# alex-ozdemir/collaborative-zksnark

Measured on AMD Instinct MI355X. Metric: collaborative Groth16 proofs/sec (BLS12-377, 2^20 constraints, SPDZ N=2), higher is better.
Workload: dtype u32

## Files before the change

collaborative-zksnark_amd/csrc/core.hip:

```cpp
#include <string.h>
#include "czk_internal.h"

#include <stdlib.h>
#include <unistd.h>

namespace {
struct HwQueueDefault {
    HwQueueDefault() { setenv("GPU_MAX_HW_QUEUES", "8", 0); }
} g_hw_queue_default;
}

namespace czk {

int set_err(czk_ctx* ctx, int code, const std::string& msg) {
    if (ctx) ctx->err = msg;
    return code;
}

int ensure_buf(czk_ctx* ctx, DeviceBuf& b, size_t bytes) {
    if (b.bytes >= bytes) return CZK_OK;
    if (b.p) {
        CZK_HIP(ctx, hipStreamSynchronize(ctx->stream));
        CZK_HIP(ctx, hipFree(b.p));
        b.p = nullptr;
// ... 340 lines not shown
    (void)hipSetDevice(ctx->device);
    (void)hipStreamSynchronize(ctx->stream);
    for (auto& kv : ctx->domains) {
        DomainTables& d = kv.second;
        if (d.tw_fwd) (void)hipFree(d.tw_fwd);
        if (d.tw_inv) (void)hipFree(d.tw_inv);
        if (d.coset_fwd) (void)hipFree(d.coset_fwd);
        if (d.coset_inv) (void)hipFree(d.coset_inv);
        if (d.twu_fwd) (void)hipFree(d.twu_fwd);
        if (d.twu_inv) (void)hipFree(d.twu_inv);
        if (d.cosetu_fwd) (void)hipFree(d.cosetu_fwd);
        if (d.cosetu_inv) (void)hipFree(d.cosetu_inv);
    }
    for (auto& kv : ctx->mixed_domains) {
        MixedDomain& d = kv.second;
        if (d.tw_fwd) (void)hipFree(d.tw_fwd);
        if (d.tw_inv) (void)hipFree(d.tw_inv);
        if (d.coset_fwd) (void)hipFree(d.coset_fwd);
        if (d.coset_inv) (void)hipFree(d.coset_inv);
    }
    if (ctx->mixed_scratch.p) (void)hipFree(ctx->mixed_scratch.p);
    if (ctx->ntt_scratch.p) (void)hipFree(ctx->ntt_scratch.p);
    if (ctx->poly_scratch.p) (void)hipFree(ctx->poly_scratch.p);
    if (ctx->open_bad) (void)hipFree(ctx->open_bad);
    for (auto& b : ctx->stage_pool) (void)hipFree(b.p);
    ctx->stage_pool.clear();
    if (ctx->share_tab.p) (void)hipFree(ctx->share_tab.p);
    msm_pipeline_destroy(ctx);
    xfer_destroy(ctx);
    prof_resolve(ctx);
    for (hipEvent_t e : ctx->event_pool) (void)hipEventDestroy(e);
    if (ctx->prof_base) (void)hipEventDestroy(ctx->prof_base);
    if (ctx->own_stream) (void)hipStreamDestroy(ctx->stream);
    delete ctx;
}

namespace {
struct OptDesc {
    const char* name;
    long lo, hi;
    bool before_pipeline;
    void (*set)(czk_ctx*, long);
};
const OptDesc OPTIONS[] = {
    {"msm_slots", 1, czk_ctx::MSM_SLOTS, true, [](czk_ctx* c, long v) { c->msm_slots_in_use = (int)v; }},
    {"msm_stream_priority", 0, 2, true, [](czk_ctx* c, long v) { c->msm_stream_prio = (int)v; }},
    {"msm_lane_interleave", 0, 64, false, [](czk_ctx* c, long v) { c->msm_lane_interleave = (int)v; }},
    {"msm_sort_reuse", 0, 1, false, [](czk_ctx* c, long v) { c->msm_sort_reuse = v != 0; }},
    {"msm_sort_onepass", 0, 1, false, [](czk_ctx* c, long v) { c->msm_sort_onepass = v != 0; }},
    {"msm_fixed_c", 0, 1, false, [](czk_ctx* c, long v) { c->msm_fixed_c = v != 0; }},
    {"msm_window_g1", 0, 22, false, [](czk_ctx* c, long v) { c->msm_c_g1 = (unsigned)v; }},
    {"msm_window_g2", 0, 22, false, [](czk_ctx* c, long v) { c->msm_c_g2 = (unsigned)v; }},
    {"ntt_gen1", 0, 1, false, [](czk_ctx* c, long v) { c->ntt_gen1 = v != 0; }},
    {"ntt_fuse_pairs", 0, 1, false, [](czk_ctx* c, long v) { c->ntt_fuse_pairs = v != 0; }},
    {"net_create_timeout_ms", 0, 3600000, false, [](czk_ctx* c, long v) { c->net_create_timeout_ms = v; }},
#ifdef CZK_LAB
    {"msm_affine_rounds", 0, 3, false, [](czk_ctx* c, long v) { c->msm_affine_rounds = (unsigned)v; }},
    {"msm_reduce_sat", 0, 1, false, [](czk_ctx* c, long v) { c->msm_reduce_sat = v != 0; }},
    {"msm_reduce_sat_g2", 0, 1, false, [](czk_ctx* c, long v) { c->msm_reduce_sat_g2 = v != 0; }},
    {"msm_g2_mode", 0, 2, false, [](czk_ctx* c, long v) { c->msm_g2_mode = (int)v; }},
    {"msm_sat", 0, 1, false, [](czk_ctx* c, long v) { c->msm_sat = v != 0; }},
    {"msm_sat_g2", 0, 1, false, [](czk_ctx* c, long v) { c->msm_sat_g2 = v != 0; }},
    {"msm_no_te", 0, 1, false, [](czk_ctx* c, long v) { c->msm_no_te = v != 0; }},
    {"chaos", 0, 0x7fffffff, false, [](czk_ctx* c, long v) { c->chaos = v ? ((unsigned long long)v * 0x9E3779B97F4A7C15ull) ^ ((unsigned long long)getpid() << 32) ^ (unsigned long long)(uintptr_t)c : 0; }},
    {"chaos_drop_wait", 0, 1, false, [](czk_ctx* c, long v) { c->chaos_drop_wait = (int)v; }},
    {"ntt_skip_coset_first", 0, 1, false, [](czk_ctx* c, long v) { c->ntt_skip_coset_first = v != 0; }},
    {"msm_sort_reuse_any_inf", 0, 1, false, [](czk_ctx* c, long v) { c->msm_sort_reuse_any_inf = v != 0; }},

#endif
};
}
extern "C" int czk_ctx_set_option(czk_ctx* ctx, const char* name, long value) {
    if (!ctx || !name) return CZK_ERR_ARG;
    for (const OptDesc& o : OPTIONS) {
        if (strcmp(o.name, name) != 0) continue;
        if (value < o.lo || value > o.hi || (!strncmp(name, "msm_window", 10) && value != 0 && value < 8))
            return set_err(ctx, CZK_ERR_ARG, std::string("czk_ctx_set_option: value out of range for ") + name);
        if (o.before_pipeline && ctx->s_sort) return set_err(ctx, CZK_ERR_ARG, std::string("czk_ctx_set_option: ") + name + " must be set before the context's first MSM");
        CZK_HIP(ctx, hipStreamSynchronize(ctx->stream));
        CZK_TRY(msm_pipeline_sync(ctx));
        o.set(ctx, value);
        return CZK_OK;
    }
#ifdef CZK_LAB
    return set_err(ctx, CZK_ERR_ARG, std::string("czk_ctx_set_option: unknown option \"") + name + "\" (lab build)");
#else
    return set_err(ctx, CZK_ERR_ARG, std::string("czk_ctx_set_option: unknown option \"") + name + "\" (product build: the switches of the rejected variants exist in libczk_hip_lab.so only)");
#endif
}
extern "C" int czk_build_is_lab(void) {
#ifdef CZK_LAB
    return 1;
#else
    return 0;
#endif
}

extern "C" int czk_ctx_reserve(czk_ctx* ctx, unsigned ntt_log_d, size_t ntt_lanes, const czk_bases* bases, size_t n_scalars, size_t msm_lanes) {
    if (!ctx) return CZK_ERR_ARG;
    CZK_HIP(ctx, hipSetDevice(ctx->device));
    if (ntt_lanes) CZK_TRY(ntt_reserve(ctx, ntt_log_d, ntt_lanes));
    if (bases && msm_lanes) CZK_TRY(msm_reserve(ctx, bases, n_scalars, msm_lanes));
    return CZK_OK;
}
extern "C" void* czk_ctx_stream(const czk_ctx* ctx) { return ctx ? (void*)ctx->stream : nullptr; }
extern "C" int czk_ctx_sync(czk_ctx* ctx) {
// ... 65 lines not shown
```

collaborative-zksnark_amd/csrc/czk_internal.h:

```cpp
#pragma once
#include <hip/hip_runtime.h>

#include <atomic>
#include <map>
#include <mutex>
#include <string>
#include <vector>

#include "../../include/czk.h"
#include "curve.h"

namespace czk {

struct DomainTables {
    unsigned log_d = 0;
    u64* tw_fwd = nullptr;
    u64* tw_inv = nullptr;
    u64* coset_fwd = nullptr;
    u64* coset_inv = nullptr;
    uint32_t *twu_fwd = nullptr, *twu_inv = nullptr, *cosetu_fwd = nullptr, *cosetu_inv = nullptr;
    Fr size_inv, group_gen, group_gen_inv, generator, generator_inv, vanishing_inv;
};

struct MixedDomain {
// ... 53 lines not shown
    unsigned split_W = 0, c = 0;
    int group = 0;
    size_t lanes = 0;
};
struct CtxMark {
    uint64_t id = 0;
    hipEvent_t ev_stream = nullptr, ev_red = nullptr;
    uint64_t upto = 0;
};
}

#ifndef CZK_ACC_INTERLEAVE_DEFAULT
#define CZK_ACC_INTERLEAVE_DEFAULT 4u
#endif
struct czk_ctx {
    std::vector<czk::DeviceBuf> stage_pool;
    char* xfer_pinned[2] = {nullptr, nullptr};
    hipEvent_t xfer_ev[2] = {nullptr, nullptr};
    bool xfer_busy[2] = {false, false};
    hipStream_t s_sort = nullptr, s_acc = nullptr, s_red = nullptr;
    hipEvent_t ev_in = nullptr;
    static constexpr int MSM_SLOTS = 4;
    czk::MsmSlot msm_slots[MSM_SLOTS];
    int msm_next_slot = 0;
    uint64_t msm_seq = 0, msm_leader_seq = 0;
    int msm_slots_in_use = 4;
    char* msm_pinned = nullptr;
    size_t msm_pinned_bytes = 0, msm_pinned_used = 0;
    std::vector<czk::MsmPending> msm_pending;
    uint64_t msm_delivered = 0;
    std::vector<czk::CtxMark> marks;
    uint64_t next_mark = 1;
    std::vector<hipEvent_t> mark_events;
    bool msm_sort_reuse = false;
    bool msm_sort_reuse_any_inf = false;
    bool msm_sort_onepass = false;
    bool msm_fixed_c = false;
    unsigned msm_c_g1 = 0, msm_c_g2 = 0;
    bool msm_launch_split = false;
    int msm_lane_interleave = 0;
    int msm_stream_prio = 0;
    unsigned msm_affine_rounds = 0;
    bool msm_reduce_sat = false;
    bool msm_reduce_sat_g2 = false;
    int msm_g2_mode = 0;
    bool msm_sat = false, msm_sat_g2 = false;
    bool msm_no_te = false;
    long net_create_timeout_ms = 0;
    unsigned long long* open_bad = nullptr;
    bool ntt_skip_coset_first = false;
    unsigned long long chaos = 0;
    int chaos_drop_wait = 0;
    bool ntt_fuse_pairs = false;
    bool ntt_gen1 = false;
    bool profiling = false;
    std::map<std::string, czk::ProfEntry> prof;
    std::vector<hipEvent_t> event_pool;
    hipEvent_t prof_base = nullptr;
    int device = 0;
    hipStream_t stream = nullptr;
    bool own_stream = false;
    std::string err;
    std::map<unsigned, czk::DomainTables> domains;
    std::map<unsigned, czk::MixedDomain> mixed_domains;
    czk::DeviceBuf mixed_scratch;
    czk::DeviceBuf ntt_scratch;
    czk::DeviceBuf poly_scratch;
    czk::DeviceBuf share_tab;
    int num_cu = 256;
    size_t lds_per_block = 64 * 1024;
};

struct czk_table_set {
    unsigned c = 0, W = 0;
    size_t cover = 0;
    uint64_t* pts = nullptr;
    uint8_t* inf = nullptr;
};

struct czk_bases {
    static constexpr int MAX_EXTRA = 12;
    czk_table_set extra[MAX_EXTRA];
    std::atomic<int> n_extra{0};
    std::atomic<unsigned> nomem_class{0};
    std::mutex build_mu;
    bool per_call_width = true;
    int device = 0;
    int group = 1;
    size_t n = 0;
    unsigned c = 0;
    unsigned W = 0;
    bool unsat = false;
    bool te = false;
    bool check_wanted = false;
    bool checked = false;
    size_t n_bad = 0;
    bool te_wanted = true;
    uint64_t* pts_sw0 = nullptr;
    bool split = false;
    uint64_t* pts = nullptr;
    uint8_t* inf = nullptr;
    static constexpr size_t INF_LIST_MAX = 4096;
    bool inf_listed = false;
    std::vector<uint32_t> inf_idx;
};

// ... 168 lines not shown
```

collaborative-zksnark_amd/csrc/ntt.hip:

```cpp
#include <atomic>
#include <condition_variable>
#include <mutex>
#include <thread>

#include "czk_internal.h"
#include "ntt_pass.h"

namespace czk {

__device__ __forceinline__ Fr lds_get(const uint4* s, unsigned idx) {
    uint4 a = s[2 * idx], b = s[2 * idx + 1];
    Fr r;
    r.l[0] = a.x; r.l[1] = a.y; r.l[2] = a.z; r.l[3] = a.w;
    r.l[4] = b.x; r.l[5] = b.y; r.l[6] = b.z; r.l[7] = b.w;
    return r;
}
__device__ __forceinline__ void lds_put(uint4* s, unsigned idx, const Fr& v) {
    s[2 * idx] = make_uint4(v.l[0], v.l[1], v.l[2], v.l[3]);
    s[2 * idx + 1] = make_uint4(v.l[4], v.l[5], v.l[6], v.l[7]);
}
__device__ __forceinline__ Fr gfr_load(const u64* base, size_t idx) { return fp_load<FrParams>(base + 4 * idx); }
__device__ __forceinline__ void gfr_store(u64* base, size_t idx, const Fr& v) { fp_store<FrParams>(base + 4 * idx, v); }

__device__ __forceinline__ unsigned bitrev(unsigned v, unsigned bits) {
// ... 249 lines not shown
    d.generator_inv = fp_inv(d.generator);
    d.vanishing_inv = fp_inv(fp_sub(fp_pow_u64(d.generator, D), Fr::one()));
    ctx->domains[log_d] = d;
    *out = &ctx->domains[log_d];
    return CZK_OK;
}

constexpr unsigned NTT2_MIN_LOG = 11;

static int ensure_tables(czk_ctx* ctx, DomainTables* d, bool need_coset_fwd, bool need_coset_inv) {
    const unsigned n = d->log_d;
    const size_t D = (size_t)1 << n;
    if ((!d->tw_fwd || !d->tw_inv) && n > 0) {
        StageRoots hr[2];
        for (unsigned s = 0; s < n; s++) {
            Fr wf = d->group_gen, wi = d->group_gen_inv;
            for (unsigned k = 0; k < n - 1 - s; k++) {
                wf = fp_sqr(wf);
                wi = fp_sqr(wi);
            }
            hr[0].w[s] = wf;
            hr[1].w[s] = wi;
        }
        StageRoots* dr = nullptr;
        CZK_HIP(ctx, hipMalloc(&dr, sizeof(hr)));
        CZK_HIP(ctx, hipMemcpyAsync(dr, hr, sizeof(hr), hipMemcpyHostToDevice, ctx->stream));
        if (alloc_table_pair(ctx, &d->tw_fwd, &d->tw_inv, (D - 1 ? D - 1 : 1) * 32) != CZK_OK) {
            (void)hipFree(dr);
            return CZK_ERR_NOMEM;
        }
        size_t chunks = (D - 1 + 63) / 64;
        unsigned blocks = (unsigned)((chunks + 127) / 128);
        hipLaunchKernelGGL(k_twiddle_table, dim3(blocks), dim3(128), 0, ctx->stream, d->tw_fwd, n, dr);
        hipLaunchKernelGGL(k_twiddle_table, dim3(blocks), dim3(128), 0, ctx->stream, d->tw_inv, n, dr + 1);
        hipError_t e = hipGetLastError();
        if (e == hipSuccess) e = hipStreamSynchronize(ctx->stream);
        (void)hipFree(dr);
        if (e != hipSuccess) return drop_table_pair(ctx, &d->tw_fwd, &d->tw_inv, e);
    }
    size_t chunks = (D + 63) / 64;
    unsigned blocks = (unsigned)((chunks + 127) / 128);
    if (need_coset_fwd && !d->coset_fwd) {
        CZK_HIP(ctx, hipMalloc(&d->coset_fwd, D * 32));
        hipLaunchKernelGGL(k_pow_table, dim3(blocks), dim3(128), 0, ctx->stream, d->coset_fwd, D, d->generator, Fr::one());
        CZK_HIP(ctx, hipGetLastError());
    }
    if (need_coset_inv && !d->coset_inv) {
        CZK_HIP(ctx, hipMalloc(&d->coset_inv, D * 32));
        hipLaunchKernelGGL(k_pow_table, dim3(blocks), dim3(128), 0, ctx->stream, d->coset_inv, D, d->generator_inv, d->size_inv);
        CZK_HIP(ctx, hipGetLastError());
    }
    if (n >= NTT2_MIN_LOG) {
        if (!d->twu_fwd || !d->twu_inv) {
            CZK_TRY(alloc_table_pair(ctx, &d->twu_fwd, &d->twu_inv, (D - 1) * 36));
            launch_table_to_u(ctx->stream, d->tw_fwd, D - 1, d->twu_fwd);
            launch_table_to_u(ctx->stream, d->tw_inv, D - 1, d->twu_inv);
            hipError_t e = hipGetLastError();
            if (e != hipSuccess) return drop_table_pair(ctx, &d->twu_fwd, &d->twu_inv, e);
        }
        if (need_coset_fwd && !d->cosetu_fwd) {
            CZK_HIP(ctx, hipMalloc(&d->cosetu_fwd, D * 36));
            launch_table_to_u(ctx->stream, d->coset_fwd, D, d->cosetu_fwd);
            CZK_HIP(ctx, hipGetLastError());
        }
        if (need_coset_inv && !d->cosetu_inv) {
            CZK_HIP(ctx, hipMalloc(&d->cosetu_inv, D * 36));
            launch_table_to_u(ctx->stream, d->coset_inv, D, d->cosetu_inv);
            CZK_HIP(ctx, hipGetLastError());
        }
    }
    return CZK_OK;
}

int ntt_device(czk_ctx* ctx, u64* data, unsigned log_d, size_t lanes, int kind, size_t in_len, const u64* src, size_t src_stride) {
    if (kind < 0 || kind > 3) return set_err(ctx, CZK_ERR_ARG, "bad ntt kind");
    if (!src) {
        src = data;
        src_stride = (size_t)1 << log_d;
    }
    DomainTables* d = nullptr;
    CZK_TRY(get_domain(ctx, log_d, &d));
    const size_t D = (size_t)1 << log_d;
    if (in_len > D) return set_err(ctx, CZK_ERR_SIZE, "coeffs.len() > domain size (radix2/mod.rs:100)");
    if (lanes == 0) return CZK_OK;
    if (log_d > 30) return set_err(ctx, CZK_ERR_SIZE, "domain above 2^30 exceeds this build's table budget");
    const bool inverse = (kind == CZK_IFFT || kind == CZK_COSET_IFFT);
    CZK_TRY(ensure_tables(ctx, d, kind == CZK_COSET_FFT, kind == CZK_COSET_IFFT));

    const unsigned n = log_d;
    unsigned m = n == 0 ? 1 : (n + 6) / 7;
    unsigned groups[8];
    for (unsigned i = 0; i < m; i++) groups[i] = n / m + (i < n % m ? 1 : 0);

    PassArgs a;
    a.tw = inverse ? d->tw_inv : d->tw_fwd;
    a.n = n;
    a.in_len = in_len;
    a.lane_stride = D;
    a.in_lane_stride = src_stride;
    a.postconst = d->size_inv;

    u64* scratch = nullptr;
    if (m > 1) {
        CZK_TRY(ensure_buf(ctx, ctx->ntt_scratch, lanes * D * (n >= NTT2_MIN_LOG ? NTT2_SCRATCH_ELEM_BYTES : 32)));
        scratch = (u64*)ctx->ntt_scratch.p;
    }
    unsigned s_hi_plus1 = n;
    if (n >= NTT2_MIN_LOG && !ctx->ntt_gen1) {
        Pass2Args b;
        b.tw = inverse ? d->twu_inv : d->twu_fwd;
        b.n = n;
        b.in_len = in_len;
        b.lane_stride = D;
        b.in_lane_stride = src_stride;
        b.postconst = host_fr_to_u(d->size_inv);
        for (unsigned p = 0; p < m; p++) {
            const bool first = (p == 0), last = (p == m - 1);
            const unsigned K = groups[p];
            b.s_lo = s_hi_plus1 - K;
// ... 347 lines not shown
```

collaborative-zksnark_amd/csrc/ntt_pass.h:

```cpp
#pragma once
#include "czk_internal.h"
#include "fru.h"

namespace czk {

constexpr int NTT2_SCRATCH_FORMAT = 2;
constexpr bool NTT2_LAZY_SCRATCH = NTT2_SCRATCH_FORMAT == 1;
constexpr bool NTT2_SCRATCH_2R = NTT2_SCRATCH_FORMAT != 0;
constexpr size_t NTT2_SCRATCH_ELEM_BYTES = NTT2_LAZY_SCRATCH ? 36 : 32;

struct Pass2Args {
    const u64* in;
    u64* out;
    const u32* tw;
    const u32* prescale;
    const u32* posttab;
    FrU postconst;
    int post_mode;
    unsigned n;
    unsigned s_lo;
    size_t in_len;
    int first;
    size_t lane_stride;
    size_t in_lane_stride;
};

int launch_ntt2_pass(czk_ctx* ctx, const Pass2Args& a, unsigned K, bool last, size_t lanes);
int launch_ntt2_final_first(czk_ctx* ctx, const Pass2Args& ai, const Pass2Args& af, unsigned C, size_t lanes);
void launch_table_to_u(hipStream_t st, const u64* sat, size_t count, u32* dst);
FrU host_fr_to_u(const Fr& sat);

}
```

collaborative-zksnark_amd/csrc/ntt_pass.hip:

```cpp
#include "ntt_pass.h"

namespace czk {

__device__ __forceinline__ FrU tab_load(const u32* tab, size_t idx) {
    FrU r;
    const u32* p = tab + 9 * idx;
#pragma unroll
    for (int i = 0; i < 9; i++) r.l[i] = p[i];
    return r;
}

template <int K, int U>
__device__ __forceinline__ void bfly(FrU& a, FrU& b, const FrU& w) {
    FrU d = fru_sub<K, U>(a, b);
    a = fru_add(a, b);
    b = fru_mul(d, w);
}

template <int KB>
__device__ __forceinline__ void radix8(FrU* x, const FrU* tw) {
#pragma unroll
    for (int k = 0; k < 4; k++) bfly<KB, 1>(x[k], x[k + 4], tw[k]);
    bfly<2 * KB, 2>(x[0], x[2], tw[4]);
    bfly<2 * KB, 2>(x[1], x[3], tw[5]);
    bfly<2, 1>(x[4], x[6], tw[4]);
    bfly<2, 1>(x[5], x[7], tw[5]);
    x[0] = fru_normalize(x[0]);
    x[1] = fru_normalize(x[1]);
    bfly<4 * KB, 1>(x[0], x[1], tw[6]);
    bfly<2, 1>(x[2], x[3], tw[6]);
    bfly<4, 2>(x[4], x[5], tw[6]);
    bfly<2, 1>(x[6], x[7], tw[6]);
    x[0] = fru_normalize(x[0]);
    x[2] = fru_normalize(x[2]);
    x[4] = fru_normalize(x[4]);
    x[6] = fru_normalize(x[6]);
}
template <int KB>
__device__ __forceinline__ void radix4(FrU* x, const FrU* tw) {
    bfly<KB, 1>(x[0], x[2], tw[0]);
    bfly<KB, 1>(x[1], x[3], tw[1]);
    bfly<2 * KB, 2>(x[0], x[1], tw[2]);
    bfly<2, 1>(x[2], x[3], tw[2]);
    x[0] = fru_normalize(x[0]);
    x[2] = fru_normalize(x[2]);
}

template <int KB>
__device__ __forceinline__ void radix4_last(FrU* x, const FrU& tw1) {
    const FrU d02 = fru_sub<KB, 1>(x[0], x[2]);
    const FrU s02 = fru_add(x[0], x[2]);
    bfly<KB, 1>(x[1], x[3], tw1);
    x[0] = fru_normalize(fru_add(s02, x[1]));
    x[1] = fru_normalize(fru_sub<2 * KB, 2>(s02, x[1]));
    x[2] = fru_normalize(fru_add(d02, x[3]));
    x[3] = fru_normalize(fru_sub<2, 1>(d02, x[3]));
}
template <int KB>
__device__ __forceinline__ void radix8_last(FrU* x, const FrU* tw2, const FrU& tw1) {
    const FrU d04 = fru_sub<KB, 1>(x[0], x[4]);
    x[0] = fru_add(x[0], x[4]);
#pragma unroll
    for (int k = 1; k < 4; k++) bfly<KB, 1>(x[k], x[k + 4], tw2[k]);
    const FrU d = fru_sub<2 * KB, 2>(x[0], x[2]);
    x[0] = fru_add(x[0], x[2]);
    x[2] = d;
    bfly<2 * KB, 2>(x[1], x[3], tw1);
    const FrU e = fru_sub<2, 1>(d04, x[6]);
    x[4] = fru_add(d04, x[6]);
    x[6] = e;
    bfly<2, 1>(x[5], x[7], tw1);
    x[0] = fru_normalize(x[0]);
    x[1] = fru_normalize(x[1]);
    const FrU s01 = fru_add(x[0], x[1]);
    x[1] = fru_normalize(fru_sub<4 * KB, 1>(x[0], x[1]));
    x[0] = fru_normalize(s01);
    const FrU s23 = fru_add(x[2], x[3]);
    x[3] = fru_normalize(fru_sub<2, 1>(x[2], x[3]));
    x[2] = fru_normalize(s23);
    const FrU s45 = fru_add(x[4], x[5]);
    x[5] = fru_normalize(fru_sub<4, 2>(x[4], x[5]));
    x[4] = fru_normalize(s45);
    const FrU s67 = fru_add(x[6], x[7]);
    x[7] = fru_normalize(fru_sub<2, 1>(x[6], x[7]));
    x[6] = fru_normalize(s67);
}

constexpr unsigned NTT2_LOGT = 4, NTT2_T = 16;

template <int NE>
__device__ __forceinline__ FrU lds_get9(const u32* s, unsigned e) {
    FrU r;
#pragma unroll
    for (int i = 0; i < 9; i++) r.l[i] = s[i * NE + e];
    return r;
}
template <int NE>
__device__ __forceinline__ void lds_put9(u32* s, unsigned e, const FrU& v) {
#pragma unroll
    for (int i = 0; i < 9; i++) s[i * NE + e] = v.l[i];
}

template <bool LAZY_IN>
__device__ __forceinline__ FrU load_input(const Pass2Args& a, const u64* in, size_t gi) {
    if constexpr (LAZY_IN && NTT2_LAZY_SCRATCH) return tab_load((const u32*)in, gi);
    if (a.first && gi >= a.in_len) {
        FrU z;
#pragma unroll
        for (int i = 0; i < 9; i++) z.l[i] = 0;
        return z;
    }
    FrU v = fru_unpack(fp_load<FrParams>(in + 4 * gi));
    if (a.prescale) v = fru_mul(v, tab_load(a.prescale, gi));
    return v;
}
__device__ __forceinline__ void store_output(const Pass2Args& a, u64* out, size_t k, const FrU& v, bool last) {
    if (!last && NTT2_SCRATCH_2R && !NTT2_LAZY_SCRATCH) {
        fp_store<FrParams>(out + 4 * k, fru_pack(fru_reduce_2r(v)));
        return;
    }
    if (!last && NTT2_LAZY_SCRATCH) {
        const FrU t = fru_reduce_2r(v);
        u32* p = (u32*)out + 9 * k;
#pragma unroll
        for (int i = 0; i < 9; i++) p[i] = t.l[i];
        return;
    }
    Fr s;
    if (last && a.post_mode == 1) s = fru_canon_mulout(fru_mul(v, a.postconst));
    else if (last && a.post_mode == 2) s = fru_canon_mulout(fru_mul(v, tab_load(a.posttab, k)));
    else s = fru_canon(v);
    fp_store<FrParams>(out + 4 * k, s);
}

template <int K, int B0, int RB, int KB, bool FROM_GLOBAL, bool TO_GLOBAL, bool LAZY_IN>
__device__ __forceinline__ void strided_step(const Pass2Args& a, u32* smem, const u64* in, u64* out, size_t base, unsigned low0) {
    constexpr int NE = (1 << K) * NTT2_T, R = 1 << RB, GROUPS = 8 / R, NTHR = NE / 8;
    const unsigned u = threadIdx.x;
#pragma unroll
    for (int g = 0; g < GROUPS; g++) {
        const unsigned gid = u + g * NTHR;
        const unsigned t = gid & (NTT2_T - 1), ro = gid >> NTT2_LOGT;
        const unsigned r_below = ro & ((1u << B0) - 1u), r_above = ro >> B0;
        const unsigned r0 = (r_above << (B0 + RB)) | r_below;
        FrU x[R];
#pragma unroll
        for (int k = 0; k < R; k++) {
            const unsigned r = r0 | ((unsigned)k << B0);
            if constexpr (FROM_GLOBAL) x[k] = load_input<LAZY_IN>(a, in, base | ((size_t)r << a.s_lo) | t);
            else x[k] = lds_get9<NE>(smem, r * NTT2_T + t);
        }
        const size_t col = (size_t)low0 | t;
        if constexpr (RB == 3) {
            FrU tw[7];
            {
                const unsigned q = B0 + 2, s = a.s_lo + q;
                const u32* tws = a.tw + 9 * (((size_t)1 << s) - 1);
#pragma unroll
                for (int k = 0; k < 4; k++) tw[k] = tab_load(tws, (((size_t)(r_below | ((unsigned)k << B0))) << a.s_lo) | col);
            }
            {
                const unsigned q = B0 + 1, s = a.s_lo + q;
                const u32* tws = a.tw + 9 * (((size_t)1 << s) - 1);
#pragma unroll
                for (int k = 0; k < 2; k++) tw[4 + k] = tab_load(tws, (((size_t)(r_below | ((unsigned)k << B0))) << a.s_lo) | col);
            }
            {
                const unsigned s = a.s_lo + B0;
                tw[6] = tab_load(a.tw + 9 * (((size_t)1 << s) - 1), ((size_t)r_below << a.s_lo) | col);
            }
            radix8<KB>(x, tw);
        } else {
            FrU tw[3];
            {
                const unsigned q = B0 + 1, s = a.s_lo + q;
                const u32* tws = a.tw + 9 * (((size_t)1 << s) - 1);
#pragma unroll
                for (int k = 0; k < 2; k++) tw[k] = tab_load(tws, (((size_t)(r_below | ((unsigned)k << B0))) << a.s_lo) | col);
            }
            {
                const unsigned s = a.s_lo + B0;
                tw[2] = tab_load(a.tw + 9 * (((size_t)1 << s) - 1), ((size_t)r_below << a.s_lo) | col);
            }
            radix4<KB>(x, tw);
        }
#pragma unroll
        for (int k = 0; k < R; k++) {
            const unsigned r = r0 | ((unsigned)k << B0);
            if constexpr (TO_GLOBAL) store_output(a, out, base | ((size_t)r << a.s_lo) | t, x[k], false);
            else lds_put9<NE>(smem, r * NTT2_T + t, x[k]);
        }
    }
}

template <int K, bool LAZY_IN>
__global__ __launch_bounds__((1 << K) * 2) void k_ntt2_strided(Pass2Args a) {
    extern __shared__ __attribute__((aligned(16))) u32 smem2[];
    const unsigned lb_bits = a.s_lo - NTT2_LOGT;
    const unsigned B = blockIdx.x;
    const unsigned Lb = B & ((1u << lb_bits) - 1u);
    const size_t H = B >> lb_bits;
    const size_t base = (H << (a.s_lo + K)) | ((size_t)Lb << NTT2_LOGT);
    const unsigned low0 = Lb << NTT2_LOGT;
    constexpr int W = LAZY_IN ? 2 : 1;
    const u64* in = (const u64*)((const char*)a.in + (a.first ? 32 * a.in_lane_stride : (LAZY_IN ? NTT2_SCRATCH_ELEM_BYTES : 32) * a.lane_stride) * blockIdx.y);
    u64* out = (u64*)((char*)a.out + NTT2_SCRATCH_ELEM_BYTES * a.lane_stride * blockIdx.y);
    if constexpr (K == 7) {
        strided_step<7, 4, 3, 2 * W, true, false, LAZY_IN>(a, smem2, in, out, base, low0);
        __syncthreads();
        strided_step<7, 2, 2, 16 * W, false, false, LAZY_IN>(a, smem2, in, out, base, low0);
        __syncthreads();
        strided_step<7, 0, 2, 64 * W, false, true, LAZY_IN>(a, smem2, in, out, base, low0);
    } else if constexpr (K == 6) {
        strided_step<6, 3, 3, 2 * W, true, false, LAZY_IN>(a, smem2, in, out, base, low0);
        __syncthreads();
        strided_step<6, 0, 3, 16 * W, false, true, LAZY_IN>(a, smem2, in, out, base, low0);
    } else {
        strided_step<5, 2, 3, 2 * W, true, false, LAZY_IN>(a, smem2, in, out, base, low0);
        __syncthreads();
        strided_step<5, 0, 2, 16 * W, false, true, LAZY_IN>(a, smem2, in, out, base, low0);
    }
}

template <int C, int B0, int RB, int KB, bool FROM_GLOBAL, bool TO_GLOBAL>
__device__ __forceinline__ void final_step(const Pass2Args& a, u32* smem, const u64* in, u64* out, unsigned blk) {
    constexpr int LEN = 1 << C, RS = LEN + 1, NEL = RS * NTT2_T, R = 1 << RB, GROUPS = 8 / R, NTHR = LEN * NTT2_T / 8;
    constexpr int OB = C - RB;
    const unsigned hb = a.n - C;
    const unsigned u = threadIdx.x;
#pragma unroll
    for (int g = 0; g < GROUPS; g++) {
        const unsigned gid = u + g * NTHR;
        unsigned t, lo;
        if constexpr (TO_GLOBAL) {
            t = gid & (NTT2_T - 1);
            lo = gid >> NTT2_LOGT;
        } else {
            lo = gid & ((1u << OB) - 1u);
            t = gid >> OB;
        }
        const unsigned l_below = lo & ((1u << B0) - 1u), l_above = lo >> B0;
        const unsigned l0 = (l_above << (B0 + RB)) | l_below;
        const size_t chunk = (size_t)blk * NTT2_T + t;
        const size_t h = hb ? (size_t)(__brev((unsigned)chunk) >> (32 - hb)) : 0;
        FrU x[R];
#pragma unroll
        for (int k = 0; k < R; k++) {
            const unsigned l = l0 | ((unsigned)k << B0);
            if constexpr (FROM_GLOBAL) x[k] = load_input<NTT2_SCRATCH_2R>(a, in, (h << C) | l);
            else x[k] = lds_get9<NEL>(smem, t * RS + l);
        }
        if constexpr (B0 == 0) {
            const u32* tw_s1 = a.tw + 9 * 1;
            if constexpr (RB == 3) {
                FrU tw2[4];
#pragma unroll
                for (int k = 1; k < 4; k++) tw2[k] = tab_load(a.tw + 9 * 3, k);
                radix8_last<KB>(x, tw2, tab_load(tw_s1, 1));
            } else {
                radix4_last<KB>(x, tab_load(tw_s1, 1));
            }
        } else if constexpr (RB == 3) {
            FrU tw[7];
#pragma unroll
            for (int k = 0; k < 4; k++) tw[k] = tab_load(a.tw + 9 * (((size_t)1 << (B0 + 2)) - 1), l_below | ((unsigned)k << B0));
#pragma unroll
            for (int k = 0; k < 2; k++) tw[4 + k] = tab_load(a.tw + 9 * (((size_t)1 << (B0 + 1)) - 1), l_below | ((unsigned)k << B0));
            tw[6] = tab_load(a.tw + 9 * (((size_t)1 << B0) - 1), l_below);
            radix8<KB>(x, tw);
        } else {
            FrU tw[3];
#pragma unroll
            for (int k = 0; k < 2; k++) tw[k] = tab_load(a.tw + 9 * (((size_t)1 << (B0 + 1)) - 1), l_below | ((unsigned)k << B0));
            tw[2] = tab_load(a.tw + 9 * (((size_t)1 << B0) - 1), l_below);
            radix4<KB>(x, tw);
        }
#pragma unroll
        for (int k = 0; k < R; k++) {
            const unsigned l = l0 | ((unsigned)k << B0);
            if constexpr (TO_GLOBAL) {
                const size_t ko = ((size_t)(__brev(l) >> (32 - C)) << hb) | chunk;
                store_output(a, out, ko, x[k], true);
            } else {
                lds_put9<NEL>(smem, t * RS + l, x[k]);
            }
        }
    }
}

template <int C>
__global__ __launch_bounds__((1 << C) * 2) void k_ntt2_final(Pass2Args a) {
    extern __shared__ __attribute__((aligned(16))) u32 smem2[];
    constexpr int W = NTT2_SCRATCH_2R ? 2 : 1;
    const u64* in = (const u64*)((const char*)a.in + NTT2_SCRATCH_ELEM_BYTES * a.lane_stride * blockIdx.y);
    u64* out = a.out + 4 * a.lane_stride * blockIdx.y;
    if constexpr (C == 7) {
        final_step<7, 4, 3, 2 * W, true, false>(a, smem2, in, out, blockIdx.x);
        __syncthreads();
        final_step<7, 2, 2, 16 * W, false, false>(a, smem2, in, out, blockIdx.x);
        __syncthreads();
        final_step<7, 0, 2, 64 * W, false, true>(a, smem2, in, out, blockIdx.x);
    } else if constexpr (C == 6) {
        final_step<6, 3, 3, 2 * W, true, false>(a, smem2, in, out, blockIdx.x);
        __syncthreads();
        final_step<6, 0, 3, 16 * W, false, true>(a, smem2, in, out, blockIdx.x);
    } else {
        final_step<5, 2, 3, 2 * W, true, false>(a, smem2, in, out, blockIdx.x);
        __syncthreads();
        final_step<5, 0, 2, 16 * W, false, true>(a, smem2, in, out, blockIdx.x);
    }
}

template <int C, int RB, int KB>
__device__ __forceinline__ void final_step_keep(const Pass2Args& ai, const Pass2Args& af, const u32* smem, unsigned blk, FrU* y) {
    constexpr int LEN = 1 << C, RS = LEN + 1, NEL = RS * NTT2_T, R = 1 << RB, GROUPS = 8 / R, NTHR = LEN * NTT2_T / 8;
    const unsigned hb = ai.n - C;
    const unsigned u = threadIdx.x;
#pragma unroll
    for (int g = 0; g < GROUPS; g++) {
        const unsigned gid = u + g * NTHR;
        const unsigned t = gid & (NTT2_T - 1), lo = gid >> NTT2_LOGT;
        const unsigned l0 = lo << RB;
        const size_t chunk = (size_t)blk * NTT2_T + t;
        FrU x[R];
#pragma unroll
        for (int k = 0; k < R; k++) x[k] = lds_get9<NEL>(smem, t * RS + (l0 | (unsigned)k));
        const u32* tw_s1 = ai.tw + 9 * 1;
        if constexpr (RB == 3) {
            FrU tw2[4];
#pragma unroll
            for (int k = 1; k < 4; k++) tw2[k] = tab_load(ai.tw + 9 * 3, k);
            radix8_last<KB>(x, tw2, tab_load(tw_s1, 1));
        } else {
            radix4_last<KB>(x, tab_load(tw_s1, 1));
        }
#pragma unroll
        for (int k = 0; k < R; k++) {
            const unsigned l = l0 | (unsigned)k;
            const size_t ko = ((size_t)(__brev(l) >> (32 - C)) << hb) | chunk;
            const Fr s = fru_canon_mulout(fru_mul(x[k], ai.postconst));
            y[g * R + k] = fru_mul(fru_unpack(s), tab_load(af.prescale, ko));
        }
    }
}
template <int C, int RB>
__device__ __forceinline__ void final_put_strided(u32* smem, const FrU* y) {
    constexpr int LEN = 1 << C, NE = LEN * NTT2_T, R = 1 << RB, GROUPS = 8 / R, NTHR = LEN * NTT2_T / 8;
    const unsigned u = threadIdx.x;
#pragma unroll
    for (int g = 0; g < GROUPS; g++) {
        const unsigned gid = u + g * NTHR;
        const unsigned t = gid & (NTT2_T - 1), l0 = (gid >> NTT2_LOGT) << RB;
#pragma unroll
        for (int k = 0; k < R; k++) lds_put9<NE>(smem, (__brev(l0 | (unsigned)k) >> (32 - C)) * NTT2_T + t, y[g * R + k]);
    }
}
template <int C>
__global__ __launch_bounds__((1 << C) * 2) void k_ntt2_final_first(Pass2Args ai, Pass2Args af) {
    extern __shared__ __attribute__((aligned(16))) u32 smem2[];
    constexpr int W = NTT2_SCRATCH_2R ? 2 : 1;
    const u64* in = (const u64*)((const char*)ai.in + NTT2_SCRATCH_ELEM_BYTES * ai.lane_stride * blockIdx.y);
    u64* out = (u64*)((char*)af.out + NTT2_SCRATCH_ELEM_BYTES * af.lane_stride * blockIdx.y);
    const unsigned blk = blockIdx.x;
    const size_t base = (size_t)blk << NTT2_LOGT;
    const unsigned low0 = blk << NTT2_LOGT;
    FrU y[8];
    if constexpr (C == 7) {
        final_step<7, 4, 3, 2 * W, true, false>(ai, smem2, in, nullptr, blk);
        __syncthreads();
        final_step<7, 2, 2, 16 * W, false, false>(ai, smem2, in, nullptr, blk);
        __syncthreads();
        final_step_keep<7, 2, 64 * W>(ai, af, smem2, blk, y);
        __syncthreads();
        final_put_strided<7, 2>(smem2, y);
        __syncthreads();
        strided_step<7, 4, 3, 2, false, false, false>(af, smem2, nullptr, out, base, low0);
        __syncthreads();
        strided_step<7, 2, 2, 16, false, false, false>(af, smem2, nullptr, out, base, low0);
        __syncthreads();
        strided_step<7, 0, 2, 64, false, true, false>(af, smem2, nullptr, out, base, low0);
    } else if constexpr (C == 6) {
        final_step<6, 3, 3, 2 * W, true, false>(ai, smem2, in, nullptr, blk);
        __syncthreads();
        final_step_keep<6, 3, 16 * W>(ai, af, smem2, blk, y);
        __syncthreads();
        final_put_strided<6, 3>(smem2, y);
        __syncthreads();
        strided_step<6, 3, 3, 2, false, false, false>(af, smem2, nullptr, out, base, low0);
        __syncthreads();
        strided_step<6, 0, 3, 16, false, true, false>(af, smem2, nullptr, out, base, low0);
    } else {
        final_step<5, 2, 3, 2 * W, true, false>(ai, smem2, in, nullptr, blk);
        __syncthreads();
        final_step_keep<5, 2, 16 * W>(ai, af, smem2, blk, y);
        __syncthreads();
        final_put_strided<5, 2>(smem2, y);
        __syncthreads();
        strided_step<5, 2, 3, 2, false, false, false>(af, smem2, nullptr, out, base, low0);
        __syncthreads();
        strided_step<5, 0, 2, 16, false, true, false>(af, smem2, nullptr, out, base, low0);
    }
}

__global__ void k_table_to_u(const u64* sat, size_t count, u32* dst) {
    size_t i = (size_t)blockIdx.x * blockDim.x + threadIdx.x;
    if (i >= count) return;
    Fr k32;
#pragma unroll
    for (int j = 0; j < 8; j++) k32.l[j] = fru_k32(j);
    FrU v = fru_unpack(fp_mul(fp_load<FrParams>(sat + 4 * i), k32));
#pragma unroll
    for (int j = 0; j < 9; j++) dst[9 * i + j] = v.l[j];
}

void launch_table_to_u(hipStream_t st, const u64* sat, size_t count, u32* dst) {
    if (!count) return;
    hipLaunchKernelGGL(k_table_to_u, dim3((unsigned)((count + 255) / 256)), dim3(256), 0, st, sat, count, dst);
}

FrU host_fr_to_u(const Fr& sat) {
    Fr k32;
    for (int j = 0; j < 8; j++) k32.l[j] = fru_k32(j);
    Fr v = fp_mul(sat, k32);
    FrU r;
    for (int i = 0; i < 9; i++) {
        const int bit = 29 * i, w = bit >> 5, off = bit & 31;
        u64 two = (u64)v.l[w] | ((w + 1) < 8 ? ((u64)v.l[w + 1] << 32) : 0);
        u32 x = (u32)(two >> off);
        r.l[i] = i < 8 ? (x & FRU_MASK) : x;
    }
    return r;
}

int launch_ntt2_final_first(czk_ctx* ctx, const Pass2Args& ai, const Pass2Args& af, unsigned C, size_t lanes) {
    const size_t D = (size_t)1 << ai.n;
    const dim3 grid((unsigned)(D >> (C + NTT2_LOGT)), (unsigned)lanes), block((1u << C) * 2);
    const size_t lds = (size_t)9 * (((size_t)1 << C) + 1) * NTT2_T * 4;
    if (lds > ctx->lds_per_block) return set_err(ctx, CZK_ERR_HIP, "fused NTT pass needs " + std::to_string(lds) + " bytes of LDS per workgroup");
    if (C == 7) hipLaunchKernelGGL(k_ntt2_final_first<7>, grid, block, lds, ctx->stream, ai, af);
    else if (C == 6) hipLaunchKernelGGL(k_ntt2_final_first<6>, grid, block, lds, ctx->stream, ai, af);
    else hipLaunchKernelGGL(k_ntt2_final_first<5>, grid, block, lds, ctx->stream, ai, af);
    CZK_HIP(ctx, hipGetLastError());
    return CZK_OK;
}

int launch_ntt2_pass(czk_ctx* ctx, const Pass2Args& a, unsigned K, bool last, size_t lanes) {
    const size_t D = (size_t)1 << a.n;
    const unsigned blocks = (unsigned)(D >> (K + NTT2_LOGT));
    const dim3 grid(blocks, (unsigned)lanes), block((1u << K) * 2);
    const size_t lds_need = last ? (size_t)9 * (((size_t)1 << K) + 1) * NTT2_T * 4 : (size_t)9 * ((size_t)1 << (K + NTT2_LOGT)) * 4;
    if (lds_need > ctx->lds_per_block)
        return set_err(ctx, CZK_ERR_HIP, "NTT pass needs " + std::to_string(lds_need) + " bytes of LDS per workgroup; this device offers " + std::to_string(ctx->lds_per_block));
    if (!last) {
        const size_t lds = (size_t)9 * ((size_t)1 << (K + NTT2_LOGT)) * 4;
        if (a.first || !NTT2_SCRATCH_2R) {
            if (K == 7) hipLaunchKernelGGL((k_ntt2_strided<7, false>), grid, block, lds, ctx->stream, a);
            else if (K == 6) hipLaunchKernelGGL((k_ntt2_strided<6, false>), grid, block, lds, ctx->stream, a);
            else hipLaunchKernelGGL((k_ntt2_strided<5, false>), grid, block, lds, ctx->stream, a);
        } else {
            if (K == 7) hipLaunchKernelGGL((k_ntt2_strided<7, true>), grid, block, lds, ctx->stream, a);
            else if (K == 6) hipLaunchKernelGGL((k_ntt2_strided<6, true>), grid, block, lds, ctx->stream, a);
            else hipLaunchKernelGGL((k_ntt2_strided<5, true>), grid, block, lds, ctx->stream, a);
        }
    } else {
        const size_t lds = (size_t)9 * (((size_t)1 << K) + 1) * NTT2_T * 4;
        if (K == 7) hipLaunchKernelGGL(k_ntt2_final<7>, grid, block, lds, ctx->stream, a);
        else if (K == 6) hipLaunchKernelGGL(k_ntt2_final<6>, grid, block, lds, ctx->stream, a);
        else hipLaunchKernelGGL(k_ntt2_final<5>, grid, block, lds, ctx->stream, a);
    }
    CZK_HIP(ctx, hipGetLastError());
    return CZK_OK;
}

}
```

Baseline: 13.35.

## Store NTT twiddles as packed 8-word entries and interleave lane groups in block order

Twiddle tables are now stored as 32-byte saturated Montgomery values instead of the 9-word 29-bit-limb form, and each tab_load unpacks on the fly. This cuts table memory traffic and gives aligned loads, at the cost of extra unpack ALU work per twiddle. Separately, NTT pass grids are flattened to 1D, and block_tile_lane maps block IDs so that runs of 8 tiles are interleaved across groups of lanes (default 4). Blocks for different lanes that share the same twiddles then run close together, which should improve cache reuse.

```diff
diff --git a/collaborative-zksnark_amd/csrc/core.hip b/collaborative-zksnark_amd/csrc/core.hip
--- a/collaborative-zksnark_amd/csrc/core.hip
+++ b/collaborative-zksnark_amd/csrc/core.hip
@@ -416,6 +416,7 @@
     {"msm_window_g1", 0, 22, false, [](czk_ctx* c, long v) { c->msm_c_g1 = (unsigned)v; }},
     {"msm_window_g2", 0, 22, false, [](czk_ctx* c, long v) { c->msm_c_g2 = (unsigned)v; }},
     {"ntt_gen1", 0, 1, false, [](czk_ctx* c, long v) { c->ntt_gen1 = v != 0; }},
+    {"ntt_lane_group", 0, 64, false, [](czk_ctx* c, long v) { c->ntt_lane_group = (unsigned)v; }},
     {"ntt_fuse_pairs", 0, 1, false, [](czk_ctx* c, long v) { c->ntt_fuse_pairs = v != 0; }},
     {"net_create_timeout_ms", 0, 3600000, false, [](czk_ctx* c, long v) { c->net_create_timeout_ms = v; }},
 #ifdef CZK_LAB
diff --git a/collaborative-zksnark_amd/csrc/czk_internal.h b/collaborative-zksnark_amd/csrc/czk_internal.h
--- a/collaborative-zksnark_amd/csrc/czk_internal.h
+++ b/collaborative-zksnark_amd/csrc/czk_internal.h
@@ -129,6 +129,7 @@
     unsigned long long chaos = 0;
     int chaos_drop_wait = 0;
     bool ntt_fuse_pairs = false;
+    unsigned ntt_lane_group = 4;
     bool ntt_gen1 = false;
     bool profiling = false;
     std::map<std::string, czk::ProfEntry> prof;
diff --git a/collaborative-zksnark_amd/csrc/ntt.hip b/collaborative-zksnark_amd/csrc/ntt.hip
--- a/collaborative-zksnark_amd/csrc/ntt.hip
+++ b/collaborative-zksnark_amd/csrc/ntt.hip
@@ -325,19 +325,19 @@
     }
     if (n >= NTT2_MIN_LOG) {
         if (!d->twu_fwd || !d->twu_inv) {
-            CZK_TRY(alloc_table_pair(ctx, &d->twu_fwd, &d->twu_inv, (D - 1) * 36));
+            CZK_TRY(alloc_table_pair(ctx, &d->twu_fwd, &d->twu_inv, (D - 1) * NTT2_TAB_ENTRY_BYTES));
             launch_table_to_u(ctx->stream, d->tw_fwd, D - 1, d->twu_fwd);
             launch_table_to_u(ctx->stream, d->tw_inv, D - 1, d->twu_inv);
             hipError_t e = hipGetLastError();
             if (e != hipSuccess) return drop_table_pair(ctx, &d->twu_fwd, &d->twu_inv, e);
         }
         if (need_coset_fwd && !d->cosetu_fwd) {
-            CZK_HIP(ctx, hipMalloc(&d->cosetu_fwd, D * 36));
+            CZK_HIP(ctx, hipMalloc(&d->cosetu_fwd, D * NTT2_TAB_ENTRY_BYTES));
             launch_table_to_u(ctx->stream, d->coset_fwd, D, d->cosetu_fwd);
             CZK_HIP(ctx, hipGetLastError());
         }
         if (need_coset_inv && !d->cosetu_inv) {
-            CZK_HIP(ctx, hipMalloc(&d->cosetu_inv, D * 36));
+            CZK_HIP(ctx, hipMalloc(&d->cosetu_inv, D * NTT2_TAB_ENTRY_BYTES));
             launch_table_to_u(ctx->stream, d->coset_inv, D, d->cosetu_inv);
             CZK_HIP(ctx, hipGetLastError());
         }
diff --git a/collaborative-zksnark_amd/csrc/ntt_pass.h b/collaborative-zksnark_amd/csrc/ntt_pass.h
--- a/collaborative-zksnark_amd/csrc/ntt_pass.h
+++ b/collaborative-zksnark_amd/csrc/ntt_pass.h
@@ -8,6 +8,10 @@
 constexpr bool NTT2_LAZY_SCRATCH = NTT2_SCRATCH_FORMAT == 1;
 constexpr bool NTT2_SCRATCH_2R = NTT2_SCRATCH_FORMAT != 0;
 constexpr size_t NTT2_SCRATCH_ELEM_BYTES = NTT2_LAZY_SCRATCH ? 36 : 32;
+
+constexpr size_t NTT2_TAB_WORDS = 8, NTT2_TAB_ENTRY_BYTES = 4 * NTT2_TAB_WORDS;
+
+constexpr unsigned NTT2_LANE_GROUP_DEFAULT = 4;
 
 struct Pass2Args {
     const u64* in;
@@ -23,6 +27,8 @@
     int first;
     size_t lane_stride;
     size_t in_lane_stride;
+    unsigned tiles, lanes;
+    unsigned lane_group;
 };
 
 int launch_ntt2_pass(czk_ctx* ctx, const Pass2Args& a, unsigned K, bool last, size_t lanes);
diff --git a/collaborative-zksnark_amd/csrc/ntt_pass.hip b/collaborative-zksnark_amd/csrc/ntt_pass.hip
--- a/collaborative-zksnark_amd/csrc/ntt_pass.hip
+++ b/collaborative-zksnark_amd/csrc/ntt_pass.hip
@@ -3,11 +3,28 @@
 namespace czk {
 
 __device__ __forceinline__ FrU tab_load(const u32* tab, size_t idx) {
+    return fru_unpack(fp_load<FrParams>((const u64*)(tab + NTT2_TAB_WORDS * idx)));
+}
+__device__ __forceinline__ FrU lazy_load(const u32* lanes, size_t idx) {
     FrU r;
-    const u32* p = tab + 9 * idx;
+    const u32* p = lanes + 9 * idx;
 #pragma unroll
     for (int i = 0; i < 9; i++) r.l[i] = p[i];
     return r;
+}
+__device__ __forceinline__ void block_tile_lane(const Pass2Args& a, unsigned& tile, unsigned& lane) {
+    if (a.lane_group == 0) {
+        tile = blockIdx.x, lane = blockIdx.y;
+        return;
+    }
+    const unsigned per_group = a.tiles * a.lane_group;
+    const unsigned q = blockIdx.x / per_group, rem = blockIdx.x - q * per_group;
+    const unsigned left = a.lanes - q * a.lane_group, g = left < a.lane_group ? left : a.lane_group;
+    const unsigned run = rem / (8 * g), r2 = rem - run * 8 * g;
+    const unsigned tleft = a.tiles - run * 8, w = tleft < 8 ? tleft : 8;
+    const unsigned li = r2 / w;
+    tile = run * 8 + (r2 - li * w);
+    lane = q * a.lane_group + li;
 }
 
 template <int K, int U>
@@ -103,7 +120,7 @@
 
 template <bool LAZY_IN>
 __device__ __forceinline__ FrU load_input(const Pass2Args& a, const u64* in, size_t gi) {
-    if constexpr (LAZY_IN && NTT2_LAZY_SCRATCH) return tab_load((const u32*)in, gi);
+    if constexpr (LAZY_IN && NTT2_LAZY_SCRATCH) return lazy_load((const u32*)in, gi);
     if (a.first && gi >= a.in_len) {
         FrU z;
 #pragma unroll
@@ -155,32 +172,32 @@
             FrU tw[7];
             {
                 const unsigned q = B0 + 2, s = a.s_lo + q;
-                const u32* tws = a.tw + 9 * (((size_t)1 << s) - 1);
+                const u32* tws = a.tw + NTT2_TAB_WORDS * (((size_t)1 << s) - 1);
 #pragma unroll
                 for (int k = 0; k < 4; k++) tw[k] = tab_load(tws, (((size_t)(r_below | ((unsigned)k << B0))) << a.s_lo) | col);
             }
             {
                 const unsigned q = B0 + 1, s = a.s_lo + q;
-                const u32* tws = a.tw + 9 * (((size_t)1 << s) - 1);
+                const u32* tws = a.tw + NTT2_TAB_WORDS * (((size_t)1 << s) - 1);
 #pragma unroll
                 for (int k = 0; k < 2; k++) tw[4 + k] = tab_load(tws, (((size_t)(r_below | ((unsigned)k << B0))) << a.s_lo) | col);
             }
             {
                 const unsigned s = a.s_lo + B0;
-                tw[6] = tab_load(a.tw + 9 * (((size_t)1 << s) - 1), ((size_t)r_below << a.s_lo) | col);
+                tw[6] = tab_load(a.tw + NTT2_TAB_WORDS * (((size_t)1 << s) - 1), ((size_t)r_below << a.s_lo) | col);
             }
             radix8<KB>(x, tw);
         } else {
             FrU tw[3];
             {
                 const unsigned q = B0 + 1, s = a.s_lo + q;
-                const u32* tws = a.tw + 9 * (((size_t)1 << s) - 1);
+                const u32* tws = a.tw + NTT2_TAB_WORDS * (((size_t)1 << s) - 1);
 #pragma unroll
                 for (int k = 0; k < 2; k++) tw[k] = tab_load(tws, (((size_t)(r_below | ((unsigned)k << B0))) << a.s_lo) | col);
             }
             {
                 const unsigned s = a.s_lo + B0;
-                tw[2] = tab_load(a.tw + 9 * (((size_t)1 << s) - 1), ((size_t)r_below << a.s_lo) | col);
+                tw[2] = tab_load(a.tw + NTT2_TAB_WORDS * (((size_t)1 << s) - 1), ((size_t)r_below << a.s_lo) | col);
             }
             radix4<KB>(x, tw);
         }
@@ -197,14 +214,15 @@
 __global__ __launch_bounds__((1 << K) * 2) void k_ntt2_strided(Pass2Args a) {
     extern __shared__ __attribute__((aligned(16))) u32 smem2[];
     const unsigned lb_bits = a.s_lo - NTT2_LOGT;
-    const unsigned B = blockIdx.x;
+    unsigned B, lane;
+    block_tile_lane(a, B, lane);
     const unsigned Lb = B & ((1u << lb_bits) - 1u);
     const size_t H = B >> lb_bits;
     const size_t base = (H << (a.s_lo + K)) | ((size_t)Lb << NTT2_LOGT);
     const unsigned low0 = Lb << NTT2_LOGT;
     constexpr int W = LAZY_IN ? 2 : 1;
-    const u64* in = (const u64*)((const char*)a.in + (a.first ? 32 * a.in_lane_stride : (LAZY_IN ? NTT2_SCRATCH_ELEM_BYTES : 32) * a.lane_stride) * blockIdx.y);
-    u64* out = (u64*)((char*)a.out + NTT2_SCRATCH_ELEM_BYTES * a.lane_stride * blockIdx.y);
+    const u64* in = (const u64*)((const char*)a.in + (a.first ? 32 * a.in_lane_stride : (LAZY_IN ? NTT2_SCRATCH_ELEM_BYTES : 32) * a.lane_stride) * lane);
+    u64* out = (u64*)((char*)a.out + NTT2_SCRATCH_ELEM_BYTES * a.lane_stride * lane);
     if constexpr (K == 7) {
         strided_step<7, 4, 3, 2 * W, true, false, LAZY_IN>(a, smem2, in, out, base, low0);
         __syncthreads();
@@ -251,11 +269,11 @@
             else x[k] = lds_get9<NEL>(smem, t * RS + l);
         }
         if constexpr (B0 == 0) {
-            const u32* tw_s1 = a.tw + 9 * 1;
+            const u32* tw_s1 = a.tw + NTT2_TAB_WORDS * 1;
             if constexpr (RB == 3) {
                 FrU tw2[4];
 #pragma unroll
-                for (int k = 1; k < 4; k++) tw2[k] = tab_load(a.tw + 9 * 3, k);
+                for (int k = 1; k < 4; k++) tw2[k] = tab_load(a.tw + NTT2_TAB_WORDS * 3, k);
                 radix8_last<KB>(x, tw2, tab_load(tw_s1, 1));
             } else {
                 radix4_last<KB>(x, tab_load(tw_s1, 1));
@@ -263,16 +281,16 @@
         } else if constexpr (RB == 3) {
             FrU tw[7];
 #pragma unroll
-            for (int k = 0; k < 4; k++) tw[k] = tab_load(a.tw + 9 * (((size_t)1 << (B0 + 2)) - 1), l_below | ((unsigned)k << B0));
-#pragma unroll
-            for (int k = 0; k < 2; k++) tw[4 + k] = tab_load(a.tw + 9 * (((size_t)1 << (B0 + 1)) - 1), l_below | ((unsigned)k << B0));
-            tw[6] = tab_load(a.tw + 9 * (((size_t)1 << B0) - 1), l_below);
+            for (int k = 0; k < 4; k++) tw[k] = tab_load(a.tw + NTT2_TAB_WORDS * (((size_t)1 << (B0 + 2)) - 1), l_below | ((unsigned)k << B0));
+#pragma unroll
+            for (int k = 0; k < 2; k++) tw[4 + k] = tab_load(a.tw + NTT2_TAB_WORDS * (((size_t)1 << (B0 + 1)) - 1), l_below | ((unsigned)k << B0));
+            tw[6] = tab_load(a.tw + NTT2_TAB_WORDS * (((size_t)1 << B0) - 1), l_below);
             radix8<KB>(x, tw);
         } else {
             FrU tw[3];
 #pragma unroll
-            for (int k = 0; k < 2; k++) tw[k] = tab_load(a.tw + 9 * (((size_t)1 << (B0 + 1)) - 1), l_below | ((unsigned)k << B0));
-            tw[2] = tab_load(a.tw + 9 * (((size_t)1 << B0) - 1), l_below);
+            for (int k = 0; k < 2; k++) tw[k] = tab_load(a.tw + NTT2_TAB_WORDS * (((size_t)1 << (B0 + 1)) - 1), l_below | ((unsigned)k << B0));
+            tw[2] = tab_load(a.tw + NTT2_TAB_WORDS * (((size_t)1 << B0) - 1), l_below);
             radix4<KB>(x, tw);
         }
 #pragma unroll
@@ -292,22 +310,24 @@
 __global__ __launch_bounds__((1 << C) * 2) void k_ntt2_final(Pass2Args a) {
     extern __shared__ __attribute__((aligned(16))) u32 smem2[];
     constexpr int W = NTT2_SCRATCH_2R ? 2 : 1;
-    const u64* in = (const u64*)((const char*)a.in + NTT2_SCRATCH_ELEM_BYTES * a.lane_stride * blockIdx.y);
-    u64* out = a.out + 4 * a.lane_stride * blockIdx.y;
+    unsigned blk, lane;
+    block_tile_lane(a, blk, lane);
+    const u64* in = (const u64*)((const char*)a.in + NTT2_SCRATCH_ELEM_BYTES * a.lane_stride * lane);
+    u64* out = a.out + 4 * a.lane_stride * lane;
     if constexpr (C == 7) {
-        final_step<7, 4, 3, 2 * W, true, false>(a, smem2, in, out, blockIdx.x);
-        __syncthreads();
-        final_step<7, 2, 2, 16 * W, false, false>(a, smem2, in, out, blockIdx.x);
-        __syncthreads();
-        final_step<7, 0, 2, 64 * W, false, true>(a, smem2, in, out, blockIdx.x);
+        final_step<7, 4, 3, 2 * W, true, false>(a, smem2, in, out, blk);
+        __syncthreads();
+        final_step<7, 2, 2, 16 * W, false, false>(a, smem2, in, out, blk);
+        __syncthreads();
+        final_step<7, 0, 2, 64 * W, false, true>(a, smem2, in, out, blk);
     } else if constexpr (C == 6) {
-        final_step<6, 3, 3, 2 * W, true, false>(a, smem2, in, out, blockIdx.x);
-        __syncthreads();
-        final_step<6, 0, 3, 16 * W, false, true>(a, smem2, in, out, blockIdx.x);
+        final_step<6, 3, 3, 2 * W, true, false>(a, smem2, in, out, blk);
+        __syncthreads();
+        final_step<6, 0, 3, 16 * W, false, true>(a, smem2, in, out, blk);
     } else {
-        final_step<5, 2, 3, 2 * W, true, false>(a, smem2, in, out, blockIdx.x);
-        __syncthreads();
-        final_step<5, 0, 2, 16 * W, false, true>(a, smem2, in, out, blockIdx.x);
+        final_step<5, 2, 3, 2 * W, true, false>(a, smem2, in, out, blk);
+        __syncthreads();
+        final_step<5, 0, 2, 16 * W, false, true>(a, smem2, in, out, blk);
     }
 }
 
@@ -325,11 +345,11 @@
         FrU x[R];
 #pragma unroll
         for (int k = 0; k < R; k++) x[k] = lds_get9<NEL>(smem, t * RS + (l0 | (unsigned)k));
-        const u32* tw_s1 = ai.tw + 9 * 1;
+        const u32* tw_s1 = ai.tw + NTT2_TAB_WORDS * 1;
         if constexpr (RB == 3) {
             FrU tw2[4];
 #pragma unroll
-            for (int k = 1; k < 4; k++) tw2[k] = tab_load(ai.tw + 9 * 3, k);
+            for (int k = 1; k < 4; k++) tw2[k] = tab_load(ai.tw + NTT2_TAB_WORDS * 3, k);
             radix8_last<KB>(x, tw2, tab_load(tw_s1, 1));
         } else {
             radix4_last<KB>(x, tab_load(tw_s1, 1));
@@ -359,9 +379,10 @@
 __global__ __launch_bounds__((1 << C) * 2) void k_ntt2_final_first(Pass2Args ai, Pass2Args af) {
     extern __shared__ __attribute__((aligned(16))) u32 smem2[];
     constexpr int W = NTT2_SCRATCH_2R ? 2 : 1;
-    const u64* in = (const u64*)((const char*)ai.in + NTT2_SCRATCH_ELEM_BYTES * ai.lane_stride * blockIdx.y);
-    u64* out = (u64*)((char*)af.out + NTT2_SCRATCH_ELEM_BYTES * af.lane_stride * blockIdx.y);
-    const unsigned blk = blockIdx.x;
+    unsigned blk, lane;
+    block_tile_lane(ai, blk, lane);
+    const u64* in = (const u64*)((const char*)ai.in + NTT2_SCRATCH_ELEM_BYTES * ai.lane_stride * lane);
+    u64* out = (u64*)((char*)af.out + NTT2_SCRATCH_ELEM_BYTES * af.lane_stride * lane);
     const size_t base = (size_t)blk << NTT2_LOGT;
     const unsigned low0 = blk << NTT2_LOGT;
     FrU y[8];
@@ -408,9 +429,7 @@
     Fr k32;
 #pragma unroll
     for (int j = 0; j < 8; j++) k32.l[j] = fru_k32(j);
-    FrU v = fru_unpack(fp_mul(fp_load<FrParams>(sat + 4 * i), k32));
-#pragma unroll
-    for (int j = 0; j < 9; j++) dst[9 * i + j] = v.l[j];
+    fp_store<FrParams>((u64*)(dst + NTT2_TAB_WORDS * i), fp_mul(fp_load<FrParams>(sat + 4 * i), k32));
 }
 
 void launch_table_to_u(hipStream_t st, const u64* sat, size_t count, u32* dst) {
@@ -432,9 +451,20 @@
     return r;
 }
 
-int launch_ntt2_final_first(czk_ctx* ctx, const Pass2Args& ai, const Pass2Args& af, unsigned C, size_t lanes) {
+static int pass_grid(czk_ctx* ctx, Pass2Args& a, size_t tiles, size_t lanes, dim3* grid) {
+    if (tiles * lanes > 0x7fffffffu) return set_err(ctx, CZK_ERR_SIZE, "NTT pass: more than 2^31 - 1 workgroups");
+    a.tiles = (unsigned)tiles, a.lanes = (unsigned)lanes;
+    a.lane_group = ctx->ntt_lane_group < lanes ? ctx->ntt_lane_group : (unsigned)lanes;
+    *grid = a.lane_group ? dim3((unsigned)(tiles * lanes)) : dim3((unsigned)tiles, (unsigned)lanes);
+    return CZK_OK;
+}
+
+int launch_ntt2_final_first(czk_ctx* ctx, const Pass2Args& ai_, const Pass2Args& af, unsigned C, size_t lanes) {
+    Pass2Args ai = ai_;
     const size_t D = (size_t)1 << ai.n;
-    const dim3 grid((unsigned)(D >> (C + NTT2_LOGT)), (unsigned)lanes), block((1u << C) * 2);
+    dim3 grid;
+    CZK_TRY(pass_grid(ctx, ai, D >> (C + NTT2_LOGT), lanes, &grid));
+    const dim3 block((1u << C) * 2);
     const size_t lds = (size_t)9 * (((size_t)1 << C) + 1) * NTT2_T * 4;
     if (lds > ctx->lds_per_block) return set_err(ctx, CZK_ERR_HIP, "fused NTT pass needs " + std::to_string(lds) + " bytes of LDS per workgroup");
     if (C == 7) hipLaunchKernelGGL(k_ntt2_final_first<7>, grid, block, lds, ctx->stream, ai, af);
@@ -444,10 +474,12 @@
     return CZK_OK;
 }
 
-int launch_ntt2_pass(czk_ctx* ctx, const Pass2Args& a, unsigned K, bool last, size_t lanes) {
+int launch_ntt2_pass(czk_ctx* ctx, const Pass2Args& a_, unsigned K, bool last, size_t lanes) {
+    Pass2Args a = a_;
     const size_t D = (size_t)1 << a.n;
-    const unsigned blocks = (unsigned)(D >> (K + NTT2_LOGT));
-    const dim3 grid(blocks, (unsigned)lanes), block((1u << K) * 2);
+    dim3 grid;
+    CZK_TRY(pass_grid(ctx, a, D >> (K + NTT2_LOGT), lanes, &grid));
+    const dim3 block((1u << K) * 2);
     const size_t lds_need = last ? (size_t)9 * (((size_t)1 << K) + 1) * NTT2_T * 4 : (size_t)9 * ((size_t)1 << (K + NTT2_LOGT)) * 4;
     if (lds_need > ctx->lds_per_block)
         return set_err(ctx, CZK_ERR_HIP, "NTT pass needs " + std::to_string(lds_need) + " bytes of LDS per workgroup; this device offers " + std::to_string(ctx->lds_per_block));
```

Result: no change. 13.40, median of 4 (+0.4%).
